# mfkiwl/hyteg

Measured on AMD Instinct MI355X. Metric: DoF-updates/s, P1 Laplace apply() level 8, higher is better.
Workload: dtype f64

## Files before the change

hyteg_amd/capi.py:

```python
from __future__ import annotations

import ctypes as C
from pathlib import Path

_PKG = Path(__file__).resolve().parent
_LIB_PATH = _PKG / "lib" / "libhyteg_hip.so"

REPLACE, ADD = 0, 1
MIN_LEVEL, MAX_LEVEL, MAX_SRCS = 2, 11, 4

_vp, _i, _d, _sz, _i64 = C.c_void_p, C.c_int, C.c_double, C.c_size_t, C.c_int64
_dp = C.POINTER(C.c_double)
SIGNATURES = {
    "hyteg_hip_version": (C.c_char_p, []),
    "hyteg_hip_last_error": (C.c_char_p, []),
    "hyteg_hip_device_count": (_i, [C.POINTER(_i)]),
    "hyteg_hip_set_device": (_i, [_i]),
    "hyteg_hip_device_name": (_i, [C.c_char_p, _sz]),
    "hyteg_hip_malloc": (_i, [C.POINTER(_vp), _sz]),
    "hyteg_hip_free": (_i, [_vp]),
    "hyteg_hip_memset_zero": (_i, [_vp, _sz, _vp]),
    "hyteg_hip_upload": (_i, [_vp, _vp, _sz, _vp]),
    "hyteg_hip_download": (_i, [_vp, _vp, _sz, _vp]),
    "hyteg_hip_copy": (_i, [_vp, _vp, _sz, _vp]),
# ... 15 lines not shown
    "hyteg_hip_event_destroy": (_i, [_vp]),
    "hyteg_hip_event_record": (_i, [_vp, _vp]),
    "hyteg_hip_stream_wait_event": (_i, [_vp, _vp]),
    "hyteg_hip_comm_available": (_i, [C.c_char_p, _sz]),
    "hyteg_hip_comm_unique_id": (_i, [C.c_char_p]),
    "hyteg_hip_comm_create": (_i, [C.POINTER(_vp), _i, _i, C.c_char_p]),
    "hyteg_hip_comm_destroy": (_i, [_vp]),
    "hyteg_hip_comm_exchange": (_i, [_vp, _i, C.POINTER(_i), _vp, C.POINTER(_i), _vp, C.POINTER(_i), _vp]),
    "hyteg_hip_comm_allreduce_sum": (_i, [_vp, _vp, _i, _vp]),
    "hyteg_hip_p2p_arena_create": (_i, [C.c_size_t, C.POINTER(_vp), C.c_char_p, C.POINTER(_i)]),
    "hyteg_hip_p2p_arena_destroy": (_i, [_vp]),
    "hyteg_hip_p2p_arena_open": (_i, [C.c_char_p, C.POINTER(_vp)]),
    "hyteg_hip_p2p_arena_close": (_i, [_vp]),
    "hyteg_hip_p2p_pack": (_i, [_vp, _i, _vp, _vp, _vp, _i, C.c_ulonglong, _vp, _vp]),
    "hyteg_hip_p2p_wait": (_i, [_vp, _i, _i, C.c_ulonglong, _vp, C.c_uint, _vp]),
    "hyteg_hip_p1_apply_cell_boundary_p2p": (_i, [_vp, _vp, _i, _vp, C.c_uint, _i, _vp, _vp, _vp, _i, C.c_ulonglong, _vp, _vp]),
    "hyteg_hip_reduce_shared_after_p2p": (_i, [_vp, _vp, _vp, _vp, _i, _i, _i, _vp, _i, _i, C.c_ulonglong, _vp, C.c_uint, _vp]),
    "hyteg_hip_graph_begin_capture": (_i, [_vp]),
    "hyteg_hip_graph_end_capture": (_i, [_vp, C.POINTER(_vp)]),
    "hyteg_hip_graph_abort_capture": (_i, [_vp]),
    "hyteg_hip_graph_launch": (_i, [_vp, _vp]),
    "hyteg_hip_graph_destroy": (_i, [_vp]),
    "hyteg_hip_prepare_level": (_i, [_i]),
    "hyteg_hip_cell_width": (_i64, [_i]),
    "hyteg_hip_cell_size": (_i64, [_i]),
    "hyteg_hip_cell_inner_size": (_i64, [_i]),
    "hyteg_hip_cell_index": (_i64, [_i, _i, _i, _i]),
    "hyteg_hip_p1_apply_cell": (_i, [_vp, _vp, _i, _dp, _i, _vp]),
    "hyteg_hip_p1_apply_cell_steps": (_i, [C.POINTER(_vp), C.POINTER(_vp), _i, _i, _dp, _i, _vp]),
    "hyteg_hip_p1_apply_kernel_name": (_i, [_i, _i, C.c_char_p, _sz]),
    "hyteg_hip_p1_residual_jacobi_start_f32": (_i, [_vp, _vp, _vp, _vp, _i, _dp, _d, _vp]),
    "hyteg_hip_p1_jacobi_accumulate_f32": (_i, [_vp, _vp, _vp, _i, _dp, _d, _vp]),
    "hyteg_hip_set_apply_shape": (_i, [_i, _i, _i]),
    "hyteg_hip_p1_apply_cell_f32": (_i, [_vp, _vp, _i, _dp, _i, _vp]),
    "hyteg_hip_p1_jacobi_cell_f32": (_i, [_vp, _vp, _vp, _vp, _i, _dp, _d, _vp]),
    "hyteg_hip_convert_f64_to_f32": (_i, [_vp, _vp, _sz, _vp]),
    "hyteg_hip_convert_f32_to_f64": (_i, [_vp, _vp, _sz, _vp]),
    "hyteg_hip_axpy_f32_into_f64": (_i, [_vp, _vp, _d, _sz, _vp]),
    "hyteg_hip_p1_jacobi_cell": (_i, [_vp, _vp, _vp, _vp, _i, _dp, _d, _vp]),
    "hyteg_hip_p1_chebyshev_start_cell": (_i, [_vp, _vp, _vp, _vp, _i, _dp, _vp]),
    "hyteg_hip_p1_chebyshev_step_cell": (_i, [_vp, _vp, _vp, _vp, _i, _dp, _d, _d, _i, _vp]),
    "hyteg_hip_p1_sor_cell": (_i, [_vp, _vp, _i, _dp, _d, _i, _vp]),
    "hyteg_hip_p1_residual_cell": (_i, [_vp, _vp, _vp, _i, _dp, _vp]),
    "hyteg_hip_p1_sor_cell_sweeps": (_i, [_vp, _vp, _i, _dp, _d, _i, _i, _vp]),
    "hyteg_hip_set_sor_algorithm": (_i, [_i]),
    "hyteg_hip_p1_assign_cell": (_i, [_vp, _i, C.POINTER(_vp), _dp, _i, _vp]),
    "hyteg_hip_p1_add_cell": (_i, [_vp, _i, C.POINTER(_vp), _dp, _i, _vp]),
    "hyteg_hip_p1_mult_cell": (_i, [_vp, _i, C.POINTER(_vp), _i, _vp]),
    "hyteg_hip_dot_workspace_bytes": (_sz, []),
    "hyteg_hip_p1_dot_cell": (_i, [_vp, _vp, _i, _vp, _vp, _vp]),
    "hyteg_hip_p1_restrict_cell": (_i, [_vp, _vp, _i, _dp, _vp]),
    "hyteg_hip_p1_prolongate_cell": (_i, [_vp, _vp, _i, _dp, _i, _vp]),
    "hyteg_hip_p1_apply_cell_boundary": (_i, [_vp, _vp, _i, _dp, C.c_uint, _i, _vp]),
    "hyteg_hip_p1_vector_cell_masked": (_i, [_i, _vp, _i, C.POINTER(_vp), _dp, _i, C.c_uint, _vp]),
    "hyteg_hip_p1_set_cell_masked": (_i, [_vp, _d, _i, C.c_uint, _vp]),
    "hyteg_hip_p1_dot_cell_masked": (_i, [_vp, _vp, _i, C.c_uint, _vp, _vp, _vp]),
    "hyteg_hip_p1_restrict_cell_masked": (_i, [_vp, _vp, _i, _dp, C.c_uint, _vp]),
    "hyteg_hip_p1_prolongate_cell_masked": (_i, [_vp, _vp, _i, _dp, C.c_uint, _vp]),
    "hyteg_hip_p1_prolongate_cell_masked_update": (_i, [_vp, _vp, _i, _dp, C.c_uint, _i, _vp]),
    "hyteg_hip_sum_shared": (_i, [_vp, _vp, _vp, _vp, _i, _i, _vp]),
    "hyteg_hip_copy_shared": (_i, [_vp, _vp, _vp, _vp, _i, _i, _vp]),
    "hyteg_hip_p1_copy_face_to_cell": (_i, [_vp, _vp, _i, _i, _i, _i, _vp]),
    "hyteg_hip_p1_copy_cell_to_face": (_i, [_vp, _vp, _i, _i, _i, _i, _i, _vp]),
    "hyteg_hip_p1_vector_cells": (_i, [_i, _i, C.POINTER(_vp), _i, C.POINTER(_vp), _dp, _i, C.POINTER(C.c_uint), _vp]),
    "hyteg_hip_p1_dot_cells": (_i, [_i, C.POINTER(_vp), C.POINTER(_vp), _i, C.POINTER(C.c_uint), _vp, _vp, _vp]),
    "hyteg_hip_p1_cg_update_cells": (_i, [_i, C.POINTER(_vp), C.POINTER(_vp), C.POINTER(_vp), C.POINTER(_vp), _d, _i, C.POINTER(C.c_uint),
# ... 184 lines not shown


def stream_wait_event(stream, ev) -> None:
    check(lib().hyteg_hip_stream_wait_event(stream, ev), "stream_wait_event")


def calib_copy(dst, src, n, nontemporal=True, stream=0) -> None:
    check(lib().hyteg_hip_calib_copy(dst, src, n, 1 if nontemporal else 0, stream), "calib_copy")


def calib_copy_ring(pairs, n, nontemporal=True, stream=0):
    m = len(pairs)
    d, s = (_vp * m)(*[p[0] for p in pairs]), (_vp * m)(*[p[1] for p in pairs])
    fn = lib().hyteg_hip_calib_copy_ring

    def call(first, count, ev_start=None, ev_stop=None):
        check(fn(d, s, m, n, 1 if nontemporal else 0, first, count, stream, ev_start, ev_stop), "calib_copy_ring")

    return call


def p1_residual_jacobi_start_f32(r_f32, e_f32, rhs, src, level, w, relax, stream=0):
    check(lib().hyteg_hip_p1_residual_jacobi_start_f32(r_f32, e_f32, rhs, src, level, _w15(w), float(relax), stream), "p1_residual_jacobi_start_f32")


def p1_jacobi_accumulate_f32(x, rhs_f32, e_f32, level, w, relax, stream=0):
    check(lib().hyteg_hip_p1_jacobi_accumulate_f32(x, rhs_f32, e_f32, level, _w15(w), float(relax), stream), "p1_jacobi_accumulate_f32")


def set_apply_shape(ny=0, lz=0, pfd=0) -> None:
    check(lib().hyteg_hip_set_apply_shape(ny, lz, pfd), "set_apply_shape")


def p1_apply_kernel_name(level, update=REPLACE) -> str:
    buf = C.create_string_buffer(256)
    check(lib().hyteg_hip_p1_apply_kernel_name(level, update, buf, 256), "p1_apply_kernel_name")
    return buf.value.decode()


def p2_prolongate_cell(fine_v, fine_e, coarse_v, coarse_e, coarse_level, update=REPLACE, mask=0x7FFF, stream=0):
    check(lib().hyteg_hip_p2_prolongate_cell(fine_v, fine_e, coarse_v, coarse_e, coarse_level, update, mask, stream), "p2_prolongate_cell")


def p2_restrict_cell(coarse_v, coarse_e, fine_v, fine_e, coarse_level, nnc, mask=0x7FFF, stream=0):
    a = (C.c_double * 14)(*[float(x) for x in nnc])
    check(lib().hyteg_hip_p2_restrict_cell(coarse_v, coarse_e, fine_v, fine_e, coarse_level, a, mask, stream), "p2_restrict_cell")


def p1_apply_cell_f32(dst, src, level, w, update=REPLACE, stream=0):
    check(lib().hyteg_hip_p1_apply_cell_f32(dst, src, level, _w15(w), update, stream), "p1_apply_cell_f32")


def p1_jacobi_cell_f32(dst, rhs, src, level, w, relax, invdiag=None, stream=0):
    check(lib().hyteg_hip_p1_jacobi_cell_f32(dst, rhs, src, invdiag, level, _w15(w), relax, stream), "p1_jacobi_cell_f32")


def convert_f64_to_f32(dst, src, n, stream=0):
    check(lib().hyteg_hip_convert_f64_to_f32(dst, src, n, stream), "convert_f64_to_f32")


def convert_f32_to_f64(dst, src, n, stream=0):
    check(lib().hyteg_hip_convert_f32_to_f64(dst, src, n, stream), "convert_f32_to_f64")


def axpy_f32_into_f64(y, x, alpha, n, stream=0):
    check(lib().hyteg_hip_axpy_f32_into_f64(y, x, alpha, n, stream), "axpy_f32_into_f64")
# ... 526 lines not shown
```

hyteg_amd/csrc/common.hpp:

```cpp
#pragma once

#include <hip/hip_runtime.h>

#include <cstdint>
#include <cstdio>
#include <cstdlib>
#include <string>

#include "../../include/hyteg_hip.h"

namespace hyteg_hip {

void set_error( const std::string& msg );
int  fail( int code, const std::string& msg );

#define HH_CHECK_HIP( expr )                                                                                         \
   do                                                                                                                \
   {                                                                                                                 \
      hipError_t _e = ( expr );                                                                                      \
      if ( _e != hipSuccess )                                                                                        \
         return ::hyteg_hip::fail( _e == hipErrorOutOfMemory ? HYTEG_HIP_ENOMEM : HYTEG_HIP_ELAUNCH,                 \
                                   std::string( #expr ) + ": " + hipGetErrorString( _e ) );                          \
   } while ( 0 )

// ... 58 lines not shown

struct Tile
{
   int a;
   int cnt;
   int z;
   int ya;
   int yb;
   int pad[3];
};
static_assert( sizeof( Tile ) == 32, "Tile must be 32 bytes" );

enum TileKind
{
   TILES_INNER = 0,
   TILES_FULL  = 1,
   TILES_ROWS  = 2
};

struct TileTable
{
   const Tile* dev   = nullptr;
   int         count = 0;
};

int get_tiles( int level, TileKind kind, int capacity, TileTable* out );

struct BrickTask;
struct BrickTable
{
   const BrickTask* dev   = nullptr;
   int              count = 0;
};
int get_bricks( int level, int NY, int LZ, BrickTable* out );

int dot_counter( hipStream_t stream, unsigned** out );

inline hipStream_t as_stream( hyteg_hip_stream_t s ) { return reinterpret_cast< hipStream_t >( s ); }

enum ApplyMode
{
   APPLY_REPLACE = 0,
   APPLY_ADD     = 1,
   APPLY_JACOBI  = 2,
   APPLY_RESIDUAL = 3,
   APPLY_RESIDUAL_F32OUT = 4,
   APPLY_JACOBI_ACCUM = 5,
   APPLY_CHEB_START = 6,
   APPLY_CHEB_STEP  = 7
};

struct Stencil15
{
   double w[15];
};
struct Nnc14
{
   double inv[14];
};

}
```

hyteg_amd/csrc/kernels_apply_zmarch.hpp:

```cpp
#pragma once

#include <algorithm>
#include <utility>
#include <vector>

#include "common.hpp"

namespace hyteg_hip {

constexpr int kBrickMaxSlices = 10;
struct BrickTask
{
   int i0;
   int W0;
   int y0;
   int xb;
   int nz;
   int pad;
   int base[kBrickMaxSlices];
};
static_assert( sizeof( BrickTask ) == 64, "BrickTask must be 64 bytes (one s_load_dwordx16)" );

struct ZMarchArgs
{
// ... 51 lines not shown
{
   int lo = __double2loint( v ), hi = __double2hiint( v );
   lo     = __builtin_amdgcn_mov_dpp( lo, 0x138, 0xf, 0xf, true );
   hi     = __builtin_amdgcn_mov_dpp( hi, 0x138, 0xf, 0xf, true );
   return __hiloint2double( hi, lo );
}
__device__ inline double zm_lane_plus_1( double v )
{
   int lo = __double2loint( v ), hi = __double2hiint( v );
   lo     = __builtin_amdgcn_mov_dpp( lo, 0x130, 0xf, 0xf, true );
   hi     = __builtin_amdgcn_mov_dpp( hi, 0x130, 0xf, 0xf, true );
   return __hiloint2double( hi, lo );
}
__device__ inline float zm_lane_minus_1( float v )
{
   return __int_as_float( __builtin_amdgcn_mov_dpp( __float_as_int( v ), 0x138, 0xf, 0xf, true ) );
}
__device__ inline float zm_lane_plus_1( float v )
{
   return __int_as_float( __builtin_amdgcn_mov_dpp( __float_as_int( v ), 0x130, 0xf, 0xf, true ) );
}

__host__ __device__ inline void zm_fill_bases( BrickTask& t, int LZ )
{
   int base = t.i0, Wq = t.W0;
   for ( int q = 0; q < kBrickMaxSlices; ++q )
   {
      t.base[q] = q < LZ + 2 ? base : 0;
      base += tri( Wq ) - ( t.y0 - 1 );
      Wq -= 1;
   }
}

template < int MODE, int NY, int LZ, int PFD, typename T >
__device__ inline void zmarch_body( const ZMarchArgs& A, const BrickTask* tasks, int ntasks, int xcd_chunk, const void* srcp, void* dstp )
{
   static_assert( LZ + 2 <= kBrickMaxSlices, "the table carries the slice bases of bricks of up to kBrickMaxSlices - 2 slices" );
   constexpr int SZ = (int) sizeof( T );
   ZM_TRACE( 0 );
   int b = blockIdx.x;
   if ( xcd_chunk > 0 )
      b = ( blockIdx.x & 7 ) * xcd_chunk + ( blockIdx.x >> 3 );
   const int task = __builtin_amdgcn_readfirstlane( b * kZMarchWavesPerBlock + ( threadIdx.x >> 6 ) );
   if ( task >= ntasks )
      return;
   const BrickTask t = tasks[task];
   const int lane = threadIdx.x & 63;
   ZM_TRACE( 1 );

   constexpr int kStAux = 2;
   const __amdgpu_buffer_rsrc_t rs = __builtin_amdgcn_make_buffer_rsrc( const_cast< void* >( srcp ), 0, A.bytes, 0x00020000 );
   const __amdgpu_buffer_rsrc_t rd = __builtin_amdgcn_make_buffer_rsrc( dstp, 0, MODE == APPLY_RESIDUAL_F32OUT ? A.bytes / 2 : A.bytes, 0x00020000 );
   constexpr bool kHasRhs = MODE == APPLY_JACOBI || MODE == APPLY_RESIDUAL || MODE == APPLY_RESIDUAL_F32OUT || MODE == APPLY_JACOBI_ACCUM ||
                            MODE == APPLY_CHEB_START;
   constexpr bool kHasInv = MODE == APPLY_JACOBI || MODE == APPLY_CHEB_START || MODE == APPLY_CHEB_STEP;
   static_assert( MODE != APPLY_CHEB_STEP || SZ == 8, "the Chebyshev step updates a double iterate" );
   const __amdgpu_buffer_rsrc_t rr = __builtin_amdgcn_make_buffer_rsrc( const_cast< void* >( kHasRhs ? A.rhs : srcp ), 0, A.bytes, 0x00020000 );
   const __amdgpu_buffer_rsrc_t rd2 =
       __builtin_amdgcn_make_buffer_rsrc( MODE == APPLY_RESIDUAL_F32OUT ? A.dst2 : dstp, 0, MODE == APPLY_RESIDUAL_F32OUT ? A.bytes / 2 : A.bytes, 0x00020000 );
   const __amdgpu_buffer_rsrc_t rx = __builtin_amdgcn_make_buffer_rsrc(
       ( MODE == APPLY_JACOBI_ACCUM || MODE == APPLY_CHEB_STEP ) ? (void*) A.xacc : dstp, 0, MODE == APPLY_JACOBI_ACCUM ? A.bytes * 2 : A.bytes, 0x00020000 );
   const __amdgpu_buffer_rsrc_t ri = __builtin_amdgcn_make_buffer_rsrc(
       const_cast< void* >( ( kHasInv && A.invdiag ) ? A.invdiag : srcp ), 0, A.bytes, 0x00020000 );

   const int lane_off = lane * SZ;
   const int ym       = t.y0 - 1;

   T S[LZ + 2][NY + 2];

   auto load_slice = [&]( auto qc, int base_q, int W_q ) {
      constexpr int q  = decltype( qc )::value;
      int           ix = base_q;
#pragma unroll
      for ( int r = 0; r < NY + 2; ++r )
      {
         const bool need = ( q == 0 ) ? ( r >= 1 ) : ( q == LZ + 1 ? ( r <= NY ) : true );
         if ( need )
         {
            const int last8 = ( W_q - ( ym + r ) - 1 - t.xb ) * SZ;
            S[q][r]         = zm_load2< T >( rs, min( lane_off, last8 ), ix * SZ );
         }
         ix += W_q - ( ym + r );
      }
   };

   int baseq[LZ + 2], Wqs[LZ + 2];
#pragma unroll
   for ( int q = 0; q < LZ + 2; ++q )
   {
      baseq[q] = t.base[q];
      Wqs[q]   = t.W0 - q;
   }
   [&]< int... Is >( std::integer_sequence< int, Is... > ) {
      ( load_slice( std::integral_constant< int, Is >{}, baseq[Is], Wqs[Is] ), ... );
   }
   ( std::make_integer_sequence < int, ( 2 + PFD <= LZ + 2 ? 2 + PFD : LZ + 2 ) > {} );
   ZM_TRACE( 2 );

   T w[15];
// ... 63 lines not shown
         T pe = w[8] * a0;
         pe        = fma( w[5], am, pe );
         pe        = fma( w[12], um, pe );
         pe        = fma( w[1], d0, pe );
         T pw = w[6] * a0;
         pw        = fma( w[13], u0, pw );
         pw        = fma( w[2], dp, pw );
         pw        = fma( w[9], ap, pw );
         T acc = zm_lane_plus_1( pe ) + zm_lane_minus_1( pw );
         acc        = fma( w[3], dp, acc );
         acc        = fma( w[10], ap, acc );
         acc        = fma( w[4], am, acc );
         acc        = fma( w[11], um, acc );
         acc        = fma( w[0], d0, acc );
         acc        = fma( w[7], a0, acc );
         acc        = fma( w[14], u0, acc );

         const int R = W - ( t.y0 + j );
         T         out;
         if ( MODE == APPLY_REPLACE )
            out = acc;
         else if ( MODE == APPLY_ADD )
            out = acc + EX0[s][j];
         else if ( MODE == APPLY_RESIDUAL || MODE == APPLY_RESIDUAL_F32OUT )
            out = EX0[s][j] - acc;
         else if ( MODE == APPLY_JACOBI_ACCUM )
            out = a0 + relax * ( invc * ( EX0[s][j] - acc ) );
         else if ( MODE == APPLY_CHEB_START )
            out = EX1[s][j] * ( EX0[s][j] - acc );
         else if ( MODE == APPLY_CHEB_STEP )
            out = EX1[s][j] * acc;
         else
            out = a0 + relax * ( EX1[s][j] * ( EX0[s][j] - acc ) );
         const int      cnt = s < t.nz ? min( 62, R - 2 - t.xb ) : 0;
         const unsigned lm1 = (unsigned) ( lane - 1 );
         const bool     on  = lm1 < (unsigned) max( cnt, 0 );
         if constexpr ( MODE == APPLY_RESIDUAL_F32OUT )
         {
            const float rf = (float) out;
            zm_store2< float, 0 >( rd, on ? lane * 4 : -8, io * 4, rf );
            zm_store2< float, 0 >( rd2, on ? lane * 4 : -8, io * 4, (float) relax * ( (float) invc * rf ) );
         }
         else if constexpr ( MODE == APPLY_JACOBI_ACCUM )
            zm_store2< double, kStAux >( rx, on ? lane * 8 : -8, io * 8, EXD[s][j] + (double) out );
         else if constexpr ( MODE == APPLY_CHEB_STEP )
         {
            double xn = EXD[s][j];
            if ( A.flag )
               xn = xn + (double) A.relax2 * (double) a0;
            xn = xn + (double) relax * (double) out;
            zm_store2< T, kStAux >( rd, on ? lane_off : -8, io * SZ, out );
            zm_store2< double, kStAux >( rx, on ? lane * 8 : -8, io * 8, xn );
         }
         else
            zm_store2< T, kStAux >( rd, on ? lane_off : -8, io * SZ, out );
         io += R;
      }
   };

   [&]< int... Is >( std::integer_sequence< int, Is... > ) { ( step( std::integral_constant< int, Is >{} ), ... ); }
   ( std::make_integer_sequence< int, LZ >{} );
   ZM_TRACE( 4 );
}

template < int MODE, int NY, int LZ, int PFD, typename T >
__global__ __launch_bounds__( 64 * kZMarchWavesPerBlock ) void p1_apply_zmarch_preload_kernel( const BrickTask* tasks, int ntasks, int xcd_chunk,
                                                                                              const ZMarchArgs A )
{
   zmarch_body< MODE, NY, LZ, PFD, T >( A, tasks, ntasks, xcd_chunk, A.src, A.dst );
}

constexpr int kZMarchMaxSteps = 16;
struct ZMarchStepPtrs
{
   const void* srcs[kZMarchMaxSteps];
   void*       dsts[kZMarchMaxSteps];
};

template < int MODE, int NY, int LZ, int PFD, typename T >
__global__ __launch_bounds__( 64 * kZMarchWavesPerBlock ) void p1_apply_zmarch_steps_kernel( const BrickTask* tasks, int ntasks, int xcd_chunk,
                                                                                            const ZMarchArgs A, const ZMarchStepPtrs P )
{
   static_assert( MODE == APPLY_REPLACE || MODE == APPLY_ADD, "a steps launch has one source and one destination per step" );
   const unsigned step = blockIdx.y < (unsigned) kZMarchMaxSteps ? blockIdx.y : 0u;
   zmarch_body< MODE, NY, LZ, PFD, T >( A, tasks, ntasks, xcd_chunk, P.srcs[step], P.dsts[step] );
}

inline void build_brick_tasks( int level, int NY, int LZ, std::vector< BrickTask >& out )
{
   const int N = ( 1 << level ) + 1;
   out.clear();
   for ( int z0 = 1; z0 <= N - 4; z0 += LZ )
   {
      const int W = N - z0;
      for ( int y0 = 1; y0 <= W - 3; y0 += NY )
      {
         const int xmax = W - y0 - 2;
         for ( int x0 = 1; x0 <= xmax; x0 += 62 )
         {
            BrickTask t{};
            t.xb = x0 - 1;
            t.y0 = y0;
            t.W0 = W + 1;
            t.i0 = slice_start( N, z0 - 1 ) + row_start( W + 1, y0 - 1 ) + t.xb;
            t.nz = std::min( LZ, N - 4 - z0 + 1 );
            zm_fill_bases( t, LZ );
            out.push_back( t );
         }
      }
   }
}

}
```

hyteg_amd/csrc/p1_apply.hip:

```cpp
#include <cstdlib>
#include <string>
#include <type_traits>

#include "kernels_apply.hpp"
#include "kernels_apply_zmarch.hpp"

using namespace hyteg_hip;

namespace {

constexpr int kTile = 1024;

struct BrickShape
{
   int  ny, lz, pfd;
   bool operator==( const BrickShape& o ) const { return ny == o.ny && lz == o.lz && pfd == o.pfd; }
};
BrickShape g_shape_override{ 0, 0, 0 };

inline BrickShape default_shape( int mode, int level, bool f32 )
{
   if ( level <= 7 )
      return ( mode == APPLY_REPLACE || f32 ) ? BrickShape{ 2, 4, 1 } : BrickShape{ 4, 4, 1 };
   if ( level == 8 )
      return ( mode == APPLY_ADD || mode == APPLY_RESIDUAL ) ? BrickShape{ 4, 8, 1 } : BrickShape{ 4, 8, 2 };
   return BrickShape{ 4, 4, 2 };
}

#define HYTEG_ZM_SHAPES( X ) X( 2, 8, 1 ) X( 4, 8, 2 ) X( 4, 8, 1 ) X( 4, 4, 2 ) X( 4, 4, 1 ) X( 2, 4, 1 ) X( 8, 4, 2 )

template < typename F >
bool with_compiled_shape( const BrickShape& s, F&& f )
{
#define HH_X( NY_, LZ_, PFD_ ) \
   if ( s == BrickShape{ NY_, LZ_, PFD_ } ) \
      return f( std::integral_constant< int, NY_ >{}, std::integral_constant< int, LZ_ >{}, std::integral_constant< int, PFD_ >{} ), true;
   HYTEG_ZM_SHAPES( HH_X )
#undef HH_X
   return false;
}

inline bool shape_compiled( const BrickShape& s )
{
   return with_compiled_shape( s, []( auto, auto, auto ) {} );
}

inline BrickShape current_shape( int mode, int level, bool f32 )
{
   static const BrickShape env = [] {
      BrickShape  e{ 0, 0, 0 };
      const char* v = getenv( "HYTEG_HIP_APPLY_SHAPE" );
      if ( v && sscanf( v, "%dx%dx%d", &e.ny, &e.lz, &e.pfd ) != 3 )
         e = BrickShape{ -1, -1, -1 };
      return e;
   }();
   if ( g_shape_override.ny )
      return g_shape_override;
   if ( env.ny )
      return env;
   return default_shape( mode, level, f32 );
}

template < typename T >
int zmarch_common_args( ZMarchArgs& A, int& nblocks, int NY, int LZ, int level, const double* w )
{
   nblocks = 0;
   BrickTable bt;
   int        rc = get_bricks( level, NY, LZ, &bt );
   if ( rc != HYTEG_HIP_OK || bt.count == 0 )
      return rc;
   A.tasks  = bt.dev;
   A.ntasks = bt.count;
   A.N      = ( 1 << level ) + 1;
   A.bytes  = (unsigned) ( tet64( A.N ) * (int64_t) sizeof( T ) );
   for ( int k = 0; k < 15; ++k )
      A.st.w[k] = w[k];
   nblocks     = ( bt.count + kZMarchWavesPerBlock - 1 ) / kZMarchWavesPerBlock;
   nblocks     = ( nblocks + 7 ) & ~7;
   A.xcd_chunk = nblocks / 8;
   static const bool xcdSlabs = env_flag( "HYTEG_HIP_APPLY_XCD_SLABS", true );
   if ( !xcdSlabs )
      A.xcd_chunk = 0;
   return HYTEG_HIP_OK;
}

template < int MODE, int NY, int LZ, int PFD, typename T >
int launch_zmarch_shape( void* dst, const T* src, const T* rhs, const T* invdiag, int level, const double* w, double relax, hipStream_t stream,
                         void* extra, double relax2, int flag )
{
   ZMarchArgs A{};
   int        nblocks = 0;
   const int  rc      = zmarch_common_args< T >( A, nblocks, NY, LZ, level, w );
   if ( rc != HYTEG_HIP_OK || nblocks == 0 )
      return rc;
   A.dst     = dst;
   A.src     = src;
   A.rhs     = rhs;
   A.invdiag = invdiag;
   A.dst2    = extra;
   A.xacc    = static_cast< double* >( extra );
   A.relax   = relax;
   A.relax2  = relax2;
   A.flag    = flag;
   hipLaunchKernelGGL( ( p1_apply_zmarch_preload_kernel< MODE, NY, LZ, PFD, T > ), dim3( nblocks ), dim3( 64 * kZMarchWavesPerBlock ), 0, stream, A.tasks,
                       A.ntasks, A.xcd_chunk, A );
   HH_CHECK_HIP( hipGetLastError() );
   return HYTEG_HIP_OK;
}

inline unsigned steps_lds_request( int level )
{
   static const int fromEnv = [] {
      const char* v = getenv( "HYTEG_HIP_APPLY_STEPS_WG_PER_CU" );
      return v ? atoi( v ) : -1;
   }();
   const int m = fromEnv >= 0 ? fromEnv : ( level == 8 ? 2 : 0 );
   return ( m >= 1 && m <= 6 ) ? (unsigned) ( ( 160 * 1024 / m ) & ~4095 ) : 0u;
}

template < int MODE, int NY, int LZ, int PFD >
int launch_zmarch_steps_shape( void* const* dsts, const void* const* srcs, int nsteps, int level, const double* w, hipStream_t stream )
{
   static_assert( MODE == APPLY_REPLACE || MODE == APPLY_ADD, "steps launch: Replace and Add" );
   ZMarchArgs A{};
   int        nblocks = 0;
   const int  rc      = zmarch_common_args< double >( A, nblocks, NY, LZ, level, w );
   if ( rc != HYTEG_HIP_OK || nblocks == 0 )
      return rc;
   ZMarchStepPtrs P{};
   for ( int k = 0; k < kZMarchMaxSteps; ++k )
   {
      P.srcs[k] = srcs[k < nsteps ? k : 0];
      P.dsts[k] = dsts[k < nsteps ? k : 0];
   }
   A.src = P.srcs[0];
   A.dst = P.dsts[0];
   auto           kern = p1_apply_zmarch_steps_kernel< MODE, NY, LZ, PFD, double >;
   const unsigned lds  = steps_lds_request( level );
   if ( lds > 0 )
   {
      static const hipError_t attr = hipFuncSetAttribute( reinterpret_cast< const void* >( kern ), hipFuncAttributeMaxDynamicSharedMemorySize, (int) lds );
      HH_CHECK_HIP( attr );
   }
   hipLaunchKernelGGL( kern, dim3( nblocks, nsteps ), dim3( 64 * kZMarchWavesPerBlock ), lds, stream, A.tasks, A.ntasks, A.xcd_chunk, A, P );
   HH_CHECK_HIP( hipGetLastError() );
   return HYTEG_HIP_OK;
}

template < int MODE, typename T = double >
int launch_zmarch( void* dst, const T* src, const T* rhs, const T* invdiag, int level, const double* w, double relax, hipStream_t stream,
                   void* extra = nullptr, double relax2 = 0.0, int flag = 0 )
{
   const int shapeMode = MODE == APPLY_RESIDUAL_F32OUT ? APPLY_RESIDUAL :
                                                         ( ( MODE == APPLY_JACOBI_ACCUM || MODE == APPLY_CHEB_START || MODE == APPLY_CHEB_STEP ) ? APPLY_JACOBI : MODE );
   int        rc       = HYTEG_HIP_OK;
   const bool compiled = with_compiled_shape( current_shape( shapeMode, level, !std::is_same< T, double >::value ), [&]( auto ny, auto lz, auto pfd ) {
      rc = launch_zmarch_shape< MODE, decltype( ny )::value, decltype( lz )::value, decltype( pfd )::value, T >( dst, src, rhs, invdiag, level, w, relax, stream,
                                                                                                                 extra, relax2, flag );
   } );
   return compiled ? rc : fail( HYTEG_HIP_EINVAL, "apply: brick shape not compiled in" );
}

template < int MODE >
int launch_zmarch_steps( void* const* dsts, const void* const* srcs, int nsteps, int level, const double* w, hipStream_t stream )
{
   int        rc       = HYTEG_HIP_OK;
   const bool compiled = with_compiled_shape( current_shape( MODE, level, false ), [&]( auto ny, auto lz, auto pfd ) {
      rc = launch_zmarch_steps_shape< MODE, decltype( ny )::value, decltype( lz )::value, decltype( pfd )::value >( dsts, srcs, nsteps, level, w, stream );
   } );
   return compiled ? rc : fail( HYTEG_HIP_EINVAL, "apply steps: brick shape not compiled in" );
}

inline bool level_runs_zmarch( int level )
{
   static const bool forceTiled = env_flag( "HYTEG_HIP_APPLY_LDS_TILED", false );
   return !forceTiled && tet64( ( 1 << level ) + 1 ) * 8 < ( (int64_t) 1 << 31 );
}

template < int MODE >
int launch_apply( double* dst, const double* src, const double* rhs, const double* invdiag, int level, const double* w,
                  double relax, hipStream_t stream )
{
   if ( level_runs_zmarch( level ) )
      return launch_zmarch< MODE >( dst, src, rhs, invdiag, level, w, relax, stream );

   TileTable tt;
   int       rc = get_tiles( level, TILES_INNER, kTile, &tt );
   if ( rc != HYTEG_HIP_OK )
      return rc;
   if ( tt.count == 0 )
      return HYTEG_HIP_OK;

   ApplyArgs A;
   A.dst     = dst;
   A.src     = src;
   A.rhs     = rhs;
   A.invdiag = invdiag;
   A.tiles   = tt.dev;
   A.ntiles  = tt.count;
   A.N       = ( 1 << level ) + 1;
   A.total   = (int) tet64( A.N );
   A.relax   = relax;
   for ( int k = 0; k < 15; ++k )
// ... 207 lines not shown
   }
   const double* s[1] = { t_out };
   return hyteg_hip_p1_add_cell( x, 1, s, &c_cur, level, stream );
}

HYTEG_HIP_API int hyteg_hip_p1_apply_kernel_name( int level, int update, char* buf, size_t buflen )
{
   HH_REQUIRE( buf && buflen > 0, "p1_apply_kernel_name: null buffer" );
   HH_REQUIRE( level_ok( level ), "p1_apply_kernel_name: level out of range [2,11]" );
   HH_REQUIRE( update == HYTEG_HIP_REPLACE || update == HYTEG_HIP_ADD, "p1_apply_kernel_name: bad update type" );
   const int mode = update == HYTEG_HIP_REPLACE ? APPLY_REPLACE : APPLY_ADD;
   if ( !level_runs_zmarch( level ) )
   {
      snprintf( buf, buflen, "p1_apply_tiled_kernel<MODE=%d>", mode );
      return HYTEG_HIP_OK;
   }
   const BrickShape s = current_shape( mode, level, false );
   snprintf( buf, buflen, "p1_apply_zmarch_preload_kernel<MODE=%d,NY=%d,LZ=%d,EX_AUX=%d,DEC=0,PFD=%d>", mode, s.ny, s.lz, mode == APPLY_ADD ? 2 : 0, s.pfd );
   return HYTEG_HIP_OK;
}

HYTEG_HIP_API int hyteg_hip_set_apply_shape( int ny, int lz, int pfd )
{
   if ( ny == 0 && lz == 0 && pfd == 0 )
   {
      g_shape_override = BrickShape{ 0, 0, 0 };
      return HYTEG_HIP_OK;
   }
   HH_REQUIRE( shape_compiled( BrickShape{ ny, lz, pfd } ), "set_apply_shape: this brick shape is not compiled in (p1_apply.hip: HYTEG_ZM_SHAPES)" );
   g_shape_override = BrickShape{ ny, lz, pfd };
   return HYTEG_HIP_OK;
}

HYTEG_HIP_API int hyteg_hip_p1_jacobi_cell( double*            dst,
                                            const double*      rhs,
                                            const double*      src,
                                            const double*      invdiag,
                                            int                level,
                                            const double*      w,
                                            double             relax,
                                            hyteg_hip_stream_t stream )
{
   HH_REQUIRE( dst && rhs && src && w, "p1_jacobi_cell: null pointer" );
   HH_REQUIRE( level_ok( level ), "p1_jacobi_cell: level out of range [2,11]" );
   HH_REQUIRE( dst != src, "p1_jacobi_cell: src and dst must not alias" );
   HH_REQUIRE( w[7] != 0.0, "p1_jacobi_cell: zero centre weight" );
   return launch_apply< APPLY_JACOBI >( dst, src, rhs, invdiag, level, w, relax, as_stream( stream ) );
}
}
```

hyteg_amd/csrc/runtime.hip:

```cpp
#include <tuple>
#include <vector>

#include "device_table.hpp"
#include "kernels_apply_zmarch.hpp"

namespace hyteg_hip {

static thread_local std::string g_last_error;

void set_error( const std::string& msg ) { g_last_error = msg; }
int  fail( int code, const std::string& msg )
{
   g_last_error = msg;
   return code;
}

static std::vector< Tile > build_tiles( int level, TileKind kind, int capacity )
{
   const int           N = ( 1 << level ) + 1;
   std::vector< Tile > tiles;
   if ( kind == TILES_ROWS )
   {
      for ( int z = 0; z < N; ++z )
         for ( int y = 0; y < N - z; ++y )
// ... 41 lines not shown
         Tile      tl{};
         tl.a   = s0 + lo;
         tl.cnt = hi - lo + 1;
         tl.z   = z;
         while ( y + 1 < W && row_start( W, y + 1 ) <= lo )
            ++y;
         tl.ya  = y;
         int yb = y;
         while ( yb + 1 < W && row_start( W, yb + 1 ) <= hi )
            ++yb;
         tl.yb = yb;
         tiles.push_back( tl );
      }
   }
   return tiles;
}

int get_tiles( int level, TileKind kind, int capacity, TileTable* out )
{
   static DeviceTableCache< std::tuple< int, int, int >, TileTable > cache;
   const TileTable*                                                   tt = nullptr;
   const int rc = cache.get( std::make_tuple( level, (int) kind, capacity ),
                             [&]( TileTable& t ) {
                                const std::vector< Tile > host = build_tiles( level, kind, capacity );
                                t.count                        = (int) host.size();
                                return upload_table( host, &t.dev );
                             },
                             &tt );
   if ( rc == HYTEG_HIP_OK )
      *out = *tt;
   return rc;
}

int get_bricks( int level, int NY, int LZ, BrickTable* out )
{
   thread_local int        lastKey[4] = { -1, -1, -1, -1 };
   thread_local BrickTable lastVal;
   int                     dev0 = 0;
   HH_CHECK_HIP( hipGetDevice( &dev0 ) );
   if ( lastKey[0] == dev0 && lastKey[1] == level && lastKey[2] == NY && lastKey[3] == LZ )
   {
      *out = lastVal;
      return HYTEG_HIP_OK;
   }
   static DeviceTableCache< std::tuple< int, int, int >, BrickTable > cache;
   const BrickTable*                                                   bt = nullptr;
   const int rc = cache.get_on( dev0, std::make_tuple( level, NY, LZ ),
                                [&]( BrickTable& b ) {
                                   std::vector< BrickTask > host;
                                   build_brick_tasks( level, NY, LZ, host );
                                   b.count = (int) host.size();
                                   return upload_table( host, &b.dev );
                                },
                                &bt );
   if ( rc != HYTEG_HIP_OK )
      return rc;
   *out       = *bt;
   lastKey[0] = dev0, lastKey[1] = level, lastKey[2] = NY, lastKey[3] = LZ;
   lastVal    = *bt;
   return HYTEG_HIP_OK;
}

}

using namespace hyteg_hip;

namespace hyteg_hip {
int dot_counter( hipStream_t stream, unsigned** out )
{
   static DeviceTableCache< hipStream_t, unsigned* > counters;
   unsigned* const*                                  c = nullptr;
   const int rc = counters.get( stream, []( unsigned*& p ) { return zeroed_table( 1, &p ); }, &c );
   if ( rc == HYTEG_HIP_OK )
      *out = *c;
   return rc;
}

int cached_operator_table( const std::vector< double >& key, const std::function< int( std::vector< double >& ) >& build, const double** dev_out )
{
   static DeviceTableCache< std::vector< double >, const double* > cache;
   const double* const*                                            t = nullptr;
   const int rc = cache.get( key,
                             [&]( const double*& dev ) {
// ... 241 lines not shown
```

include/hyteg_hip.h:

```cpp
#ifndef HYTEG_HIP_H
#define HYTEG_HIP_H

#include <stddef.h>
#include <stdint.h>

#ifdef __cplusplus
extern "C" {
#endif

#if defined( HYTEG_HIP_BUILDING )
#define HYTEG_HIP_API __attribute__( ( visibility( "default" ) ) )
#else
#define HYTEG_HIP_API
#endif

enum
{
   HYTEG_HIP_OK      = 0,
   HYTEG_HIP_EINVAL  = 1,
   HYTEG_HIP_ELAUNCH = 2,
   HYTEG_HIP_ENOMEM  = 3,
   HYTEG_HIP_ENODEV  = 4,
   HYTEG_HIP_ENOTSUP = 5
};
// ... 49 lines not shown
                                           const double*      src,
                                           int                level,
                                           const double*      w ,
                                           int                update,
                                           hyteg_hip_stream_t stream );
HYTEG_HIP_API int hyteg_hip_p1_apply_cell_steps( void* const*       dsts ,
                                                 const void* const* srcs ,
                                                 int                nsteps,
                                                 int                level,
                                                 const double*      w ,
                                                 int                update,
                                                 hyteg_hip_stream_t stream );

HYTEG_HIP_API int hyteg_hip_p1_apply_cell_f32( float* dst, const float* src, int level, const double* w , int update, hyteg_hip_stream_t stream );
HYTEG_HIP_API int hyteg_hip_p1_jacobi_cell_f32( float*             dst,
                                                const float*       rhs,
                                                const float*       src,
                                                const float*       invdiag ,
                                                int                level,
                                                const double*      w ,
                                                double             relax,
                                                hyteg_hip_stream_t stream );
HYTEG_HIP_API int hyteg_hip_convert_f64_to_f32( float* dst, const double* src, size_t n, hyteg_hip_stream_t stream );
HYTEG_HIP_API int hyteg_hip_convert_f32_to_f64( double* dst, const float* src, size_t n, hyteg_hip_stream_t stream );
HYTEG_HIP_API int hyteg_hip_axpy_f32_into_f64( double* y, const float* x, double alpha, size_t n, hyteg_hip_stream_t stream );

HYTEG_HIP_API int hyteg_hip_p1_residual_jacobi_start_f32( float* r_f32, float* e_f32, const double* rhs, const double* src, int level, const double* w,
                                                          double relax, hyteg_hip_stream_t stream );
HYTEG_HIP_API int hyteg_hip_p1_jacobi_accumulate_f32( double* x, const float* rhs_f32, const float* e_f32, int level, const double* w, double relax,
                                                      hyteg_hip_stream_t stream );

HYTEG_HIP_API int hyteg_hip_p1_apply_kernel_name( int level, int update, char* buf, size_t buflen );
HYTEG_HIP_API int hyteg_hip_set_apply_shape( int ny, int lz, int pfd );

HYTEG_HIP_API int hyteg_hip_p1_jacobi_cell( double*            dst,
                                            const double*      rhs,
                                            const double*      src,
                                            const double*      invdiag ,
                                            int                level,
                                            const double*      w ,
                                            double             relax,
                                            hyteg_hip_stream_t stream );

HYTEG_HIP_API int hyteg_hip_p1_chebyshev_start_cell( double*            t_out,
                                                     const double*      rhs,
                                                     const double*      x,
                                                     const double*      invdiag ,
                                                     int                level,
                                                     const double*      w ,
                                                     hyteg_hip_stream_t stream );
HYTEG_HIP_API int hyteg_hip_p1_chebyshev_step_cell( double*            t_out,
                                                    double*            x,
                                                    const double*      t_in,
                                                    const double*      invdiag ,
                                                    int                level,
                                                    const double*      w ,
                                                    double             c_prev,
                                                    double             c_cur,
                                                    int                has_prev,
                                                    hyteg_hip_stream_t stream );

enum hyteg_hip_sor_algorithm
{
   HYTEG_HIP_SOR_AUTO     = 0,
   HYTEG_HIP_SOR_PLANES   = 1,
   HYTEG_HIP_SOR_BLOCKS   = 2,
// ... 623 lines not shown
```

Before: 286.3 billion.

## Use aligned 56-wide store windows and 6x8 bricks for level-8 apply steps

Adds an x-stride template parameter to the z-marching apply kernel. With stride 56, each wave stores only a window aligned to 8-double boundaries of the destination, so writes cover whole 64-byte segments instead of straddling them. Level-8 Replace steps now default to this form with a new 6x8x2 brick shape. The cost is overlapping bricks: each wave still loads and computes about 62 columns but stores only 56, so some loads and arithmetic are repeated. The change also adds a host-side coverage checker and an override setter for the stride.

```diff
diff --git a/hyteg_amd/capi.py b/hyteg_amd/capi.py
--- a/hyteg_amd/capi.py
+++ b/hyteg_amd/capi.py
@@ -71,6 +71,8 @@
     "hyteg_hip_p1_residual_jacobi_start_f32": (_i, [_vp, _vp, _vp, _vp, _i, _dp, _d, _vp]),
     "hyteg_hip_p1_jacobi_accumulate_f32": (_i, [_vp, _vp, _vp, _i, _dp, _d, _vp]),
     "hyteg_hip_set_apply_shape": (_i, [_i, _i, _i]),
+    "hyteg_hip_set_apply_steps_xs": (_i, [_i]),
+    "hyteg_hip_p1_apply_brick_coverage": (_i, [_i, _i, _i, _i, _i, C.POINTER(C.c_ubyte), C.POINTER(_i)]),
     "hyteg_hip_p1_apply_cell_f32": (_i, [_vp, _vp, _i, _dp, _i, _vp]),
     "hyteg_hip_p1_jacobi_cell_f32": (_i, [_vp, _vp, _vp, _vp, _i, _dp, _d, _vp]),
     "hyteg_hip_convert_f64_to_f32": (_i, [_vp, _vp, _sz, _vp]),
@@ -321,6 +323,20 @@
     check(lib().hyteg_hip_set_apply_shape(ny, lz, pfd), "set_apply_shape")
 
 
+def set_apply_steps_xs(xs=0) -> None:
+    check(lib().hyteg_hip_set_apply_steps_xs(xs), "set_apply_steps_xs")
+
+
+def p1_apply_brick_coverage(level, ny, lz, xs=62, dst_phase=0):
+    import numpy as np
+
+    count = np.zeros(cell_size(level), dtype=np.uint8)
+    nb = _i(0)
+    check(lib().hyteg_hip_p1_apply_brick_coverage(level, ny, lz, xs, dst_phase, count.ctypes.data_as(C.POINTER(C.c_ubyte)), C.byref(nb)),
+          "p1_apply_brick_coverage")
+    return count, nb.value
+
+
 def p1_apply_kernel_name(level, update=REPLACE) -> str:
     buf = C.create_string_buffer(256)
     check(lib().hyteg_hip_p1_apply_kernel_name(level, update, buf, 256), "p1_apply_kernel_name")
diff --git a/hyteg_amd/csrc/common.hpp b/hyteg_amd/csrc/common.hpp
--- a/hyteg_amd/csrc/common.hpp
+++ b/hyteg_amd/csrc/common.hpp
@@ -114,7 +114,7 @@
    const BrickTask* dev   = nullptr;
    int              count = 0;
 };
-int get_bricks( int level, int NY, int LZ, BrickTable* out );
+int get_bricks( int level, int NY, int LZ, BrickTable* out, int XS = 62 );
 
 int dot_counter( hipStream_t stream, unsigned** out );
 
diff --git a/hyteg_amd/csrc/kernels_apply_zmarch.hpp b/hyteg_amd/csrc/kernels_apply_zmarch.hpp
--- a/hyteg_amd/csrc/kernels_apply_zmarch.hpp
+++ b/hyteg_amd/csrc/kernels_apply_zmarch.hpp
@@ -107,9 +107,20 @@
    }
 }
 
-template < int MODE, int NY, int LZ, int PFD, typename T >
+__host__ __device__ inline void zm_aligned_window( int io, int dst_phase, int R, int xb, bool live, int& lo, int& hi )
+{
+   int l = ( ( -( io + dst_phase ) - 1 ) & 7 ) + 1;
+   l     = l == 8 ? 4 : l;
+   const int end = R - 1 - xb;
+   hi            = live ? ( l + 56 < end ? l + 56 : end ) : 0;
+   lo            = xb == 0 ? 1 : l;
+   hi            = hi > lo ? hi : lo;
+}
+
+template < int MODE, int NY, int LZ, int PFD, typename T, int XS = 62 >
 __device__ inline void zmarch_body( const ZMarchArgs& A, const BrickTask* tasks, int ntasks, int xcd_chunk, const void* srcp, void* dstp )
 {
+   static_assert( XS == 62 || ( XS == 56 && ( MODE == APPLY_REPLACE || MODE == APPLY_ADD ) ), "x-stride: 62 (plain) or 56 (aligned store windows)" );
    static_assert( LZ + 2 <= kBrickMaxSlices, "the table carries the slice bases of bricks of up to kBrickMaxSlices - 2 slices" );
    constexpr int SZ = (int) sizeof( T );
    ZM_TRACE( 0 );
@@ -140,6 +151,7 @@
 
    const int lane_off = lane * SZ;
    const int ym       = t.y0 - 1;
+   const int dst_phase = XS == 56 ? (int) ( ( reinterpret_cast< uintptr_t >( dstp ) / SZ ) & 7 ) : 0;
 
    T S[LZ + 2][NY + 2];
 
@@ -269,6 +281,14 @@
             out = EX1[s][j] * acc;
          else
             out = a0 + relax * ( EX1[s][j] * ( EX0[s][j] - acc ) );
+         if constexpr ( XS == 56 )
+         {
+            int lo, hi;
+            zm_aligned_window( io, dst_phase, R, t.xb, s < t.nz, lo, hi );
+            zm_store2< T, kStAux >( rd, (unsigned) ( lane - lo ) < (unsigned) ( hi - lo ) ? lane_off : -8, io * SZ, out );
+            io += R;
+            continue;
+         }
          const int      cnt = s < t.nz ? min( 62, R - 2 - t.xb ) : 0;
          const unsigned lm1 = (unsigned) ( lane - 1 );
          const bool     on  = lm1 < (unsigned) max( cnt, 0 );
@@ -314,16 +334,16 @@
    void*       dsts[kZMarchMaxSteps];
 };
 
-template < int MODE, int NY, int LZ, int PFD, typename T >
+template < int MODE, int NY, int LZ, int PFD, typename T, int XS = 62 >
 __global__ __launch_bounds__( 64 * kZMarchWavesPerBlock ) void p1_apply_zmarch_steps_kernel( const BrickTask* tasks, int ntasks, int xcd_chunk,
                                                                                             const ZMarchArgs A, const ZMarchStepPtrs P )
 {
    static_assert( MODE == APPLY_REPLACE || MODE == APPLY_ADD, "a steps launch has one source and one destination per step" );
    const unsigned step = blockIdx.y < (unsigned) kZMarchMaxSteps ? blockIdx.y : 0u;
-   zmarch_body< MODE, NY, LZ, PFD, T >( A, tasks, ntasks, xcd_chunk, P.srcs[step], P.dsts[step] );
-}
-
-inline void build_brick_tasks( int level, int NY, int LZ, std::vector< BrickTask >& out )
+   zmarch_body< MODE, NY, LZ, PFD, T, XS >( A, tasks, ntasks, xcd_chunk, P.srcs[step], P.dsts[step] );
+}
+
+inline void build_brick_tasks( int level, int NY, int LZ, std::vector< BrickTask >& out, int XS = 62 )
 {
    const int N = ( 1 << level ) + 1;
    out.clear();
@@ -333,7 +353,7 @@
       for ( int y0 = 1; y0 <= W - 3; y0 += NY )
       {
          const int xmax = W - y0 - 2;
-         for ( int x0 = 1; x0 <= xmax; x0 += 62 )
+         for ( int x0 = 1; x0 <= xmax; x0 += XS )
          {
             BrickTask t{};
             t.xb = x0 - 1;
diff --git a/hyteg_amd/csrc/p1_apply.hip b/hyteg_amd/csrc/p1_apply.hip
--- a/hyteg_amd/csrc/p1_apply.hip
+++ b/hyteg_amd/csrc/p1_apply.hip
@@ -27,7 +27,7 @@
    return BrickShape{ 4, 4, 2 };
 }
 
-#define HYTEG_ZM_SHAPES( X ) X( 2, 8, 1 ) X( 4, 8, 2 ) X( 4, 8, 1 ) X( 4, 4, 2 ) X( 4, 4, 1 ) X( 2, 4, 1 ) X( 8, 4, 2 )
+#define HYTEG_ZM_SHAPES( X ) X( 2, 8, 1 ) X( 4, 8, 2 ) X( 4, 8, 1 ) X( 4, 4, 2 ) X( 4, 4, 1 ) X( 2, 4, 1 ) X( 8, 4, 2 ) X( 6, 8, 2 )
 
 template < typename F >
 bool with_compiled_shape( const BrickShape& s, F&& f )
@@ -45,7 +45,7 @@
    return with_compiled_shape( s, []( auto, auto, auto ) {} );
 }
 
-inline BrickShape current_shape( int mode, int level, bool f32 )
+inline bool overridden_shape( BrickShape& s )
 {
    static const BrickShape env = [] {
       BrickShape  e{ 0, 0, 0 };
@@ -55,18 +55,45 @@
       return e;
    }();
    if ( g_shape_override.ny )
-      return g_shape_override;
+      return s = g_shape_override, true;
    if ( env.ny )
-      return env;
-   return default_shape( mode, level, f32 );
+      return s = env, true;
+   return false;
+}
+inline BrickShape current_shape( int mode, int level, bool f32 )
+{
+   BrickShape s;
+   return overridden_shape( s ) ? s : default_shape( mode, level, f32 );
+}
+
+struct StepsForm
+{
+   BrickShape shape;
+   int        xs;
+};
+int g_steps_xs_override = 0;
+
+inline StepsForm steps_shape( int mode, int level )
+{
+   static const int envXs = [] {
+      const char* v = getenv( "HYTEG_HIP_APPLY_STEPS_XS" );
+      return v ? atoi( v ) : 0;
+   }();
+   StepsForm f = ( level == 8 && mode == APPLY_REPLACE ) ? StepsForm{ BrickShape{ 6, 8, 2 }, 56 } : StepsForm{ default_shape( mode, level, false ), 62 };
+   overridden_shape( f.shape );
+   if ( g_steps_xs_override )
+      f.xs = g_steps_xs_override;
+   else if ( envXs )
+      f.xs = envXs;
+   return f;
 }
 
 template < typename T >
-int zmarch_common_args( ZMarchArgs& A, int& nblocks, int NY, int LZ, int level, const double* w )
+int zmarch_common_args( ZMarchArgs& A, int& nblocks, int NY, int LZ, int level, const double* w, int XS = 62 )
 {
    nblocks = 0;
    BrickTable bt;
-   int        rc = get_bricks( level, NY, LZ, &bt );
+   int        rc = get_bricks( level, NY, LZ, &bt, XS );
    if ( rc != HYTEG_HIP_OK || bt.count == 0 )
       return rc;
    A.tasks  = bt.dev;
@@ -118,13 +145,13 @@
    return ( m >= 1 && m <= 6 ) ? (unsigned) ( ( 160 * 1024 / m ) & ~4095 ) : 0u;
 }
 
-template < int MODE, int NY, int LZ, int PFD >
+template < int MODE, int NY, int LZ, int PFD, int XS >
 int launch_zmarch_steps_shape( void* const* dsts, const void* const* srcs, int nsteps, int level, const double* w, hipStream_t stream )
 {
    static_assert( MODE == APPLY_REPLACE || MODE == APPLY_ADD, "steps launch: Replace and Add" );
    ZMarchArgs A{};
    int        nblocks = 0;
-   const int  rc      = zmarch_common_args< double >( A, nblocks, NY, LZ, level, w );
+   const int  rc      = zmarch_common_args< double >( A, nblocks, NY, LZ, level, w, XS );
    if ( rc != HYTEG_HIP_OK || nblocks == 0 )
       return rc;
    ZMarchStepPtrs P{};
@@ -135,7 +162,7 @@
    }
    A.src = P.srcs[0];
    A.dst = P.dsts[0];
-   auto           kern = p1_apply_zmarch_steps_kernel< MODE, NY, LZ, PFD, double >;
+   auto           kern = p1_apply_zmarch_steps_kernel< MODE, NY, LZ, PFD, double, XS >;
    const unsigned lds  = steps_lds_request( level );
    if ( lds > 0 )
    {
@@ -165,10 +192,14 @@
 int launch_zmarch_steps( void* const* dsts, const void* const* srcs, int nsteps, int level, const double* w, hipStream_t stream )
 {
    int        rc       = HYTEG_HIP_OK;
-   const bool compiled = with_compiled_shape( current_shape( MODE, level, false ), [&]( auto ny, auto lz, auto pfd ) {
-      rc = launch_zmarch_steps_shape< MODE, decltype( ny )::value, decltype( lz )::value, decltype( pfd )::value >( dsts, srcs, nsteps, level, w, stream );
+   const StepsForm form     = steps_shape( MODE, level );
+   const bool      compiled = ( form.xs == 56 || form.xs == 62 ) && with_compiled_shape( form.shape, [&]( auto ny, auto lz, auto pfd ) {
+      if ( form.xs == 56 )
+         rc = launch_zmarch_steps_shape< MODE, decltype( ny )::value, decltype( lz )::value, decltype( pfd )::value, 56 >( dsts, srcs, nsteps, level, w, stream );
+      else
+         rc = launch_zmarch_steps_shape< MODE, decltype( ny )::value, decltype( lz )::value, decltype( pfd )::value, 62 >( dsts, srcs, nsteps, level, w, stream );
    } );
-   return compiled ? rc : fail( HYTEG_HIP_EINVAL, "apply steps: brick shape not compiled in" );
+   return compiled ? rc : fail( HYTEG_HIP_EINVAL, "apply steps: brick shape or x-stride not compiled in" );
 }
 
 inline bool level_runs_zmarch( int level )
@@ -442,6 +473,46 @@
    return HYTEG_HIP_OK;
 }
 
+HYTEG_HIP_API int hyteg_hip_p1_apply_brick_coverage( int level, int ny, int lz, int xs, int dst_phase, unsigned char* count, int* nbricks )
+{
+   HH_REQUIRE( count && nbricks, "p1_apply_brick_coverage: null pointer" );
+   HH_REQUIRE( level >= HYTEG_HIP_MIN_LEVEL && level <= 8, "p1_apply_brick_coverage: level out of range [2,8]" );
+   HH_REQUIRE( ny >= 1 && lz >= 1 && lz + 2 <= kBrickMaxSlices && ( xs == 56 || xs == 62 ) && dst_phase >= 0 && dst_phase < 8,
+               "p1_apply_brick_coverage: bad shape, x-stride or phase" );
+   const int                N = ( 1 << level ) + 1;
+   std::vector< BrickTask > tasks;
+   build_brick_tasks( level, ny, lz, tasks, xs );
+   *nbricks = (int) tasks.size();
+   std::fill( count, count + tet64( N ), (unsigned char) 0 );
+   for ( const BrickTask& t : tasks )
+      for ( int s = 0; s < lz; ++s )
+      {
+         const int W  = t.W0 - ( s + 1 );
+         int       io = t.base[s + 1] + ( W - ( t.y0 - 1 ) );
+         for ( int j = 0; j < ny; ++j )
+         {
+            const int R  = W - ( t.y0 + j );
+            int       lo = 1, hi = 1 + std::max( s < t.nz ? std::min( 62, R - 2 - t.xb ) : 0, 0 );
+            if ( xs == 56 )
+               zm_aligned_window( io, dst_phase, R, t.xb, s < t.nz, lo, hi );
+            for ( int l = lo; l < hi; ++l )
+            {
+               HH_REQUIRE( l <= 62 && io + l >= 0 && io + l < tet64( N ), "p1_apply_brick_coverage: a store window leaves the wave or the array" );
+               count[io + l] += 1;
+            }
+            io += R;
+         }
+      }
+   return HYTEG_HIP_OK;
+}
+
+HYTEG_HIP_API int hyteg_hip_set_apply_steps_xs( int xs )
+{
+   HH_REQUIRE( xs == 0 || xs == 56 || xs == 62, "set_apply_steps_xs: the x-stride is 62 (plain), 56 (aligned store windows) or 0 (default)" );
+   g_steps_xs_override = xs;
+   return HYTEG_HIP_OK;
+}
+
 HYTEG_HIP_API int hyteg_hip_p1_jacobi_cell( double*            dst,
                                             const double*      rhs,
                                             const double*      src,
diff --git a/hyteg_amd/csrc/runtime.hip b/hyteg_amd/csrc/runtime.hip
--- a/hyteg_amd/csrc/runtime.hip
+++ b/hyteg_amd/csrc/runtime.hip
@@ -97,8 +97,10 @@
    return rc;
 }
 
-int get_bricks( int level, int NY, int LZ, BrickTable* out )
-{
+int get_bricks( int level, int NY, int LZ, BrickTable* out, int XS )
+{
+   const int rows = NY;
+   NY             = NY * 1000 + XS;
    thread_local int        lastKey[4] = { -1, -1, -1, -1 };
    thread_local BrickTable lastVal;
    int                     dev0 = 0;
@@ -113,7 +115,7 @@
    const int rc = cache.get_on( dev0, std::make_tuple( level, NY, LZ ),
                                 [&]( BrickTable& b ) {
                                    std::vector< BrickTask > host;
-                                   build_brick_tasks( level, NY, LZ, host );
+                                   build_brick_tasks( level, rows, LZ, host, XS );
                                    b.count = (int) host.size();
                                    return upload_table( host, &b.dev );
                                 },
diff --git a/include/hyteg_hip.h b/include/hyteg_hip.h
--- a/include/hyteg_hip.h
+++ b/include/hyteg_hip.h
@@ -105,6 +105,8 @@
 
 HYTEG_HIP_API int hyteg_hip_p1_apply_kernel_name( int level, int update, char* buf, size_t buflen );
 HYTEG_HIP_API int hyteg_hip_set_apply_shape( int ny, int lz, int pfd );
+HYTEG_HIP_API int hyteg_hip_set_apply_steps_xs( int xs );
+HYTEG_HIP_API int hyteg_hip_p1_apply_brick_coverage( int level, int ny, int lz, int xs, int dst_phase, unsigned char* count , int* nbricks );
 
 HYTEG_HIP_API int hyteg_hip_p1_jacobi_cell( double*            dst,
                                             const double*      rhs,
```

New measurement: 299.2 billion, median of 6. +4.5%, better.
